# yl-jiang/YOLOSeries

Measured on AMD Instinct MI355X. Metric: images/sec (640x640) YOLOv5s train-step, higher is better.
Workload: dtype bf16; 1 GPU; YOLOv5s bf16 train step (fwd+loss+bwd+clip+SGD+EMA), batch 64/GPU x 640x640 synthetic COCO-80, random-init (BASELINE.json configs[1]); global_batch=64, parallelism=dp1

## Files before the change

include/yolohip.h:

```cpp
#ifndef YOLOHIP_H
#define YOLOHIP_H

#include <stddef.h>
#include <stdint.h>

#ifdef __cplusplus
extern "C" {
#endif

typedef void* yh_stream;
typedef uint16_t yh_bf16;

enum yh_status {
    YH_OK = 0,
    YH_EINVAL = -1,
    YH_ELAUNCH = -2,
    YH_EUNSUPPORTED = -3
};

const char* yh_last_error(void);
int yh_version(void);
int yh_device_cus(void);


// ... 88 lines not shown
                          const float* ws, int C, int64_t M, float* part, yh_stream stream);
int yh_bn_bwd_finalize(const float* part, int nblk, int C, int64_t M, const float* ws,
                       float* dgamma, float* dbeta, float* coef, yh_stream stream);
int yh_bn_silu_bwd_apply(const yh_bf16* ga, int ldga, const yh_bf16* y, int ldy,
                         const float* ws, const float* gamma, const float* coef,
                         int C, int64_t M, yh_bf16* gy, int ldgy,
                         yh_bf16* gres, int ldgres, int gres_accumulate, yh_stream stream);
#define YH_BN_MAX_PARTS 4
typedef struct yh_bn_part {
    float*         ws;
    int32_t        C;
    int32_t        ldo;
    yh_bf16*       out;
    const yh_bf16* ga;
    int32_t        ldga;
    int32_t        nblk;
    const float*   gamma;
    float*         coef;
    const float*   slab;
    int32_t        ldslab;
    float          eps;
    const float*   beta;
    float*         running_mean;
    float*         running_var;
    int64_t*       num_batches;
    float          momentum;
    int32_t        _pad;
    float*         dgamma;
    float*         dbeta;
} yh_bn_part;
int yh_bn_finalize_parts(const yh_bn_part* parts, int nparts, int64_t count, yh_stream stream);
int yh_bn_bwd_finalize_parts(const yh_bn_part* parts, int nparts, int64_t M, yh_stream stream);
int yh_bn_silu_apply_parts(const yh_bf16* y, int ldy, int64_t M, const yh_bn_part* parts, int nparts, yh_stream stream);
int yh_bn_silu_bwd_apply_parts(const yh_bf16* y, int ldy, int64_t M, const yh_bn_part* parts, int nparts,
                               yh_bf16* gy, int ldgy, yh_stream stream);
int yh_colsum(const yh_bf16* g, int ldg, int C, int64_t M, float* part, float* out, yh_stream stream);

int yh_maxpool5_fwd(const yh_bf16* x, int ldx, int B, int H, int W, int C,
                    yh_bf16* out, int ldo, int8_t* idx, yh_stream stream);
int yh_maxpool5_bwd(const yh_bf16* gout, int ldgo, const int8_t* idx, int B, int H, int W, int C,
                    yh_bf16* gin, int ldgi, int accumulate, yh_stream stream);
int yh_sppf_pool3_ok(int H, int W, int C);
int yh_sppf_pool3_fwd(const yh_bf16* x, int ldx, int B, int H, int W, int C, yh_bf16* o1, yh_bf16* o2, yh_bf16* o3, int ldo,
                      int8_t* i1, int8_t* i2, int8_t* i3, yh_stream stream);
int yh_sppf_pool3_bwd(const yh_bf16* g1, const yh_bf16* g2, const yh_bf16* g3, int ldg, const int8_t* i1, const int8_t* i2, const int8_t* i3,
                      int B, int H, int W, int C, yh_bf16* gx, int ldx, int accumulate, yh_stream stream);
int yh_upsample2_bwd(const yh_bf16* ghi, int ldh, int B, int Hlo, int Wlo, int C,
                     yh_bf16* glo, int ldl, int accumulate, yh_stream stream);
int yh_input_s2d(const float* x, int B, int Cin, int H, int W, yh_bf16* out, yh_stream stream);
int yh_fill_u32(void* p, uint32_t v, int64_t n_words, yh_stream stream);

int yh_pack_bf16(const float* src, const int32_t* idx, int64_t n, yh_bf16* dst, yh_stream stream);
int yh_gather_f32(const float* src, const int32_t* idx, int64_t n, float* dst, yh_stream stream);
int yh_sgd_step(float* p, const float* g, float* buf, const uint8_t* group, int64_t n,
                const float* lr, const float* wd, int ngroups, float momentum, int nesterov,
                int first_step, const float* grad_scale, yh_stream stream);
int yh_sgd_step_dev(float* p, const float* g, float* buf, const uint8_t* group, int64_t n,
                    const float* scal, int nesterov, const float* grad_scale, yh_stream stream);
int yh_ema_update_dev(float* ema, const float* p, int64_t n, const float* decay_dev, yh_stream stream);
int yh_ema_advance(int64_t* counter, float* decay, double ratio, double tau, yh_stream stream);
int yh_sumsq(const float* x, int64_t n, float* part, float* out, yh_stream stream);
int yh_clip_scale(const float* sumsq, float max_norm, float* out, yh_stream stream);
int yh_ema_update(float* ema, const float* p, int64_t n, float decay, yh_stream stream);

typedef struct yh_v5loss_desc {
    int32_t B, maxbox, num_class, num_anchor, num_stage;
    int32_t H[4], W[4];
    float   img_size0, img_size1;
    float   anchors[4][3][2];
    float   anchor_thr;
    float   cls_smooth, cls_pos_weight, cof_pos_weight;
    int32_t use_focal; float focal_gamma, focal_alpha;
    float   iou_scale, cof_scale, cls_scale;
    int32_t pred_is_f32;
    int32_t ldp[4];
    int32_t targets_xywhn;
} yh_v5loss_desc;

size_t yh_v5loss_ws_bytes(const yh_v5loss_desc* d);
int yh_v5_assign(const yh_v5loss_desc* d, const float* targets,
                 int32_t* count, float* tbox, int32_t* tidx, void* ws, yh_stream stream);
size_t yh_v5loss_saved_bytes(const yh_v5loss_desc* d);
int yh_v5_loss_fwd(const yh_v5loss_desc* d, const void* const* preds, const float* targets,
                   double* balances, float* result, void* saved, void* ws, yh_stream stream);
int yh_v5_loss_bwd(const yh_v5loss_desc* d, const void* const* preds, const float* gout,
                   const void* saved, void* const* gpreds, void* ws, yh_stream stream);

typedef struct yh_yolox_desc {
    int32_t B, maxbox, num_class, num_stage;
    int32_t H[4], W[4], ldp[4];
    int32_t pred_is_f32;
    float   img_size0;
    int32_t use_focal; float focal_gamma, focal_alpha;
    int32_t use_l1;
    float   iou_scale, cls_scale, cof_scale, l1_scale;
    float   cls_smooth, cls_pos_weight, cof_pos_weight;
    int32_t iou_type;
    int32_t topk; float center_radius;
    float   cls_cost_const;
} yh_yolox_desc;
size_t yh_yolox_saved_bytes(const yh_yolox_desc* d);
size_t yh_yolox_ws_bytes(const yh_yolox_desc* d);
int yh_yolox_layout(const yh_yolox_desc* d, int64_t* out8);
int yh_yolox_loss_fwd(const yh_yolox_desc* d, const void* const* preds, const float* targets_xywh,
                      double* balances, float* result, void* saved, void* ws, yh_stream stream);
int yh_yolox_loss_bwd(const yh_yolox_desc* d, const void* const* preds, const float* targets_xywh, const float* gout,
// ... 43 lines not shown
```

yoloseries_amd/_lib.py:

```python
import ctypes as C
import os
import subprocess

_HERE = os.path.dirname(os.path.abspath(__file__))
LIB_PATH = os.environ.get("YH_LIBRARY") or os.path.join(_HERE, "libyolohip.so")
CSRC_DIR = os.path.join(_HERE, "csrc")


class YoloHipError(RuntimeError):
    pass


class Seg(C.Structure):
    _fields_ = [("ptr", C.c_void_p), ("ld", C.c_int32), ("C", C.c_int32), ("ups", C.c_int32), ("_pad", C.c_int32)]


class ConvDesc(C.Structure):
    _fields_ = [
        ("seg", Seg * 2), ("nseg", C.c_int32), ("mode", C.c_int32),
        ("B", C.c_int32), ("Ho", C.c_int32), ("Wo", C.c_int32),
        ("Hi", C.c_int32), ("Wi", C.c_int32),
        ("KH", C.c_int32), ("KW", C.c_int32), ("stride", C.c_int32), ("pad", C.c_int32),
        ("w", C.c_void_p), ("N", C.c_int32), ("Npad", C.c_int32),
        ("bias", C.c_void_p), ("scale", C.c_void_p), ("shift", C.c_void_p),
# ... 82 lines not shown
class Cmd(C.Structure):
    _fields_ = [("op", C.c_int32), ("nslots", C.c_int32), ("stream", C.c_int32), ("reserved", C.c_int32),
                ("slots", C.c_uint64 * YH_CMD_SLOTS)]


YH_CONV_FWD, YH_CONV_DGRAD = 0, 1
YH_ACT_NONE, YH_ACT_SILU = 0, 1

_lib = None

_vp, _i32, _i64, _f32, _sz = C.c_void_p, C.c_int32, C.c_int64, C.c_float, C.c_size_t
_SIGS = {
    "yh_last_error": (C.c_char_p, []),
    "yh_version": (_i32, []),
    "yh_device_cus": (_i32, []),
    "yh_conv_stat_blocks": (_i32, [C.POINTER(ConvDesc)]),
    "yh_conv_igemm": (_i32, [C.POINTER(ConvDesc), _vp]),
    "yh_conv_wgrad": (_i32, [C.POINTER(WgradDesc), _vp]),
    "yh_conv_wgrad_ws_bytes": (C.c_size_t, [C.POINTER(WgradDesc)]),
    "yh_conv_wgrad_patch_ok": (_i32, [C.POINTER(WgradDesc)]),
    "yh_conv_wgrad_patch_name": (_i32, [C.POINTER(WgradDesc), C.c_char_p, _i32]),
    "yh_conv_wgrad_wave_tiles": (_i32, [C.POINTER(WgradDesc)]),
    "yh_conv_wgrad_wave_name": (C.c_char_p, [C.POINTER(WgradDesc)]),
    "yh_conv_wgrad_tiles": (_i32, [_i32, _i32]),
    "yh_conv_wgrad_tiles2": (_i32, [_i32, _i32, _i32]),
    "yh_conv_wgrad_kernel_name": (C.c_char_p, [_i32, _i32]),
    "yh_conv_wgrad_kernel_name2": (C.c_char_p, [_i32, _i32, _i32]),
    "yh_conv_bnr_rows": (_i32, [C.POINTER(ConvDesc)]),
    "yh_conv_kernel_name": (_i32, [C.POINTER(ConvDesc), C.c_char_p, _i32]),
    "yh_bn_finalize": (_i32, [_vp, _i32, _i32, _i32, _i64, _vp, _vp, _vp, _vp, _vp, _f32, _f32, _vp, _vp]),
    "yh_bn_fold": (_i32, [_vp, _vp, _vp, _vp, _f32, _i32, _vp, _vp, _vp]),
    "yh_bn_frozen": (_i32, [_vp, _vp, _vp, _vp, _f32, _i32, _vp, _vp]),
    "yh_bn_fold_batch": (_i32, [_vp, _i32, _vp]),
    "yh_bn_silu_apply": (_i32, [_vp, _i32, _vp, _i32, _i64, _vp, _i32, _vp, _i32, _vp]),
    "yh_ew_blocks": (_i32, [_i64]),
    "yh_bn_silu_bwd_reduce": (_i32, [_vp, _i32, _vp, _i32, _vp, _i32, _i64, _vp, _vp]),
    "yh_bn_bwd_finalize": (_i32, [_vp, _i32, _i32, _i64, _vp, _vp, _vp, _vp, _vp]),
    "yh_bn_finalize_parts": (_i32, [_vp, _i32, _i64, _vp]),
    "yh_bn_bwd_finalize_parts": (_i32, [_vp, _i32, _i64, _vp]),
    "yh_bn_silu_apply_parts": (_i32, [_vp, _i32, _i64, _vp, _i32, _vp]),
    "yh_bn_silu_bwd_apply_parts": (_i32, [_vp, _i32, _i64, _vp, _i32, _vp, _i32, _vp]),
    "yh_bn_silu_bwd_apply": (_i32, [_vp, _i32, _vp, _i32, _vp, _vp, _vp, _i32, _i64, _vp, _i32, _vp, _i32, _i32, _vp]),
    "yh_colsum": (_i32, [_vp, _i32, _i32, _i64, _vp, _vp, _vp]),
    "yh_maxpool5_fwd": (_i32, [_vp, _i32, _i32, _i32, _i32, _i32, _vp, _i32, _vp, _vp]),
    "yh_maxpool5_bwd": (_i32, [_vp, _i32, _vp, _i32, _i32, _i32, _i32, _vp, _i32, _i32, _vp]),
    "yh_sppf_pool3_ok": (_i32, [_i32, _i32, _i32]),
    "yh_sppf_pool3_fwd": (_i32, [_vp, _i32, _i32, _i32, _i32, _i32, _vp, _vp, _vp, _i32, _vp, _vp, _vp, _vp]),
    "yh_sppf_pool3_bwd": (_i32, [_vp, _vp, _vp, _i32, _vp, _vp, _vp, _i32, _i32, _i32, _i32, _vp, _i32, _i32, _vp]),
    "yh_upsample2_bwd": (_i32, [_vp, _i32, _i32, _i32, _i32, _i32, _vp, _i32, _i32, _vp]),
    "yh_input_s2d": (_i32, [_vp, _i32, _i32, _i32, _i32, _vp, _vp]),
    "yh_fill_u32": (_i32, [_vp, C.c_uint32, _i64, _vp]),
    "yh_pack_bf16": (_i32, [_vp, _vp, _i64, _vp, _vp]),
    "yh_gather_f32": (_i32, [_vp, _vp, _i64, _vp, _vp]),
    "yh_sgd_step": (_i32, [_vp, _vp, _vp, _vp, _i64, _vp, _vp, _i32, _f32, _i32, _i32, _vp, _vp]),
    "yh_sgd_step_dev": (_i32, [_vp, _vp, _vp, _vp, _i64, _vp, _i32, _vp, _vp]),
    "yh_ema_update_dev": (_i32, [_vp, _vp, _i64, _vp, _vp]),
    "yh_ema_advance": (_i32, [_vp, _vp, C.c_double, C.c_double, _vp]),
    "yh_sumsq": (_i32, [_vp, _i64, _vp, _vp, _vp]),
    "yh_clip_scale": (_i32, [_vp, _f32, _vp, _vp]),
    "yh_ema_update": (_i32, [_vp, _vp, _i64, _f32, _vp]),
    "yh_v5loss_ws_bytes": (_sz, [C.POINTER(V5LossDesc)]),
    "yh_v5loss_saved_bytes": (_sz, [C.POINTER(V5LossDesc)]),
    "yh_v5_assign": (_i32, [C.POINTER(V5LossDesc), _vp, _vp, _vp, _vp, _vp, _vp]),
    "yh_v5_loss_fwd": (_i32, [C.POINTER(V5LossDesc), C.POINTER(_vp), _vp, _vp, _vp, _vp, _vp, _vp]),
    "yh_v5_loss_bwd": (_i32, [C.POINTER(V5LossDesc), C.POINTER(_vp), _vp, _vp, C.POINTER(_vp), _vp, _vp]),
    "yh_yolox_saved_bytes": (_sz, [C.POINTER(YoloxDesc)]),
    "yh_yolox_ws_bytes": (_sz, [C.POINTER(YoloxDesc)]),
    "yh_yolox_layout": (_i32, [C.POINTER(YoloxDesc), _vp]),
    "yh_yolox_loss_fwd": (_i32, [C.POINTER(YoloxDesc), C.POINTER(_vp), _vp, _vp, _vp, _vp, _vp, _vp]),
    "yh_yolox_loss_bwd": (_i32, [C.POINTER(YoloxDesc), C.POINTER(_vp), _vp, _vp, _vp, C.POINTER(_vp), _vp]),
    "yh_iou_matrix": (_i32, [_vp, _i32, _vp, _i32, _f32, _vp, _vp]),
    "yh_iou_pairwise": (_i32, [_i32, _vp, _vp, _i32, _vp, _vp, _vp]),
    "yh_decode_full": (_i32, [C.POINTER(DecodeDesc), C.POINTER(_vp), _vp, _vp]),
    "yh_decode_filter": (_i32, [C.POINTER(DecodeDesc), C.POINTER(_vp), _f32, _f32, _vp, _vp, _i32, _vp, _vp]),
    "yh_decode_filter_ws_bytes": (C.c_size_t, [C.POINTER(DecodeDesc)]),
    "yh_filter_decoded": (_i32, [_vp, _i32, _i32, _i32, _f32, _f32, _i32, _vp, _vp, _i32, _vp]),
    "yh_exec_op": (_i32, [C.c_char_p, C.POINTER(_i32)]),
    "yh_exec": (_i32, [C.POINTER(Cmd), _i32, C.POINTER(_vp), _i32, C.POINTER(_i32)]),
    "yh_nms_ws_bytes": (_sz, [_i32, _i32]),
    "yh_nms_batched": (_i32, [_vp, _vp, _i32, _i32, _f32, _i32, _i32, _i32, _i32, _vp, _vp, _vp, _vp, _vp]),
}
EXPORTED_SYMBOLS = tuple(_SIGS.keys())


def build(force=False):
    if force:
        subprocess.run(["make", "-C", CSRC_DIR, "clean"], check=True, stdout=subprocess.DEVNULL)
    r = subprocess.run(["make", "-C", CSRC_DIR, "-j8"], stdout=subprocess.PIPE, stderr=subprocess.STDOUT, text=True)
    if r.returncode != 0:
        raise YoloHipError("building libyolohip.so failed:\n" + r.stdout[-4000:])
    return LIB_PATH


def lib():
    global _lib
    if _lib is not None:
        return _lib
    if not os.path.exists(LIB_PATH):
        raise YoloHipError(
            f"{LIB_PATH} not found: the HIP extension is required (run __graft_entry__.build() or "
            f"`make -C {CSRC_DIR}`); there is no CPU fallback for the product path.")
    import torch
    L = C.CDLL(LIB_PATH)
    missing = []
    for name, (res, args) in _SIGS.items():
        try:
# ... 22 lines not shown
```

yoloseries_amd/csrc/arena.hip:

```cpp
#include "common.h"
#include <stdarg.h>

namespace {
constexpr int TH = 256;
inline int grid_for(long n) {
    long g = (n + TH - 1) / TH;
    if (g > 4096) g = 4096;
    if (g < 1) g = 1;
    return (int)g;
}

__global__ void pack_bf16_kernel(const float* __restrict__ src, const int32_t* __restrict__ idx, long n, uint16_t* __restrict__ dst)
{
    const long n8 = ((reinterpret_cast<uintptr_t>(dst) | reinterpret_cast<uintptr_t>(idx)) & 15) ? 0 : n >> 3;
    for (long c = (long)blockIdx.x * blockDim.x + threadIdx.x; c < n8; c += (long)gridDim.x * blockDim.x) {
        const int4 j0 = *reinterpret_cast<const int4*>(idx + c * 8), j1 = *reinterpret_cast<const int4*>(idx + c * 8 + 4);
        const int j[8] = {j0.x, j0.y, j0.z, j0.w, j1.x, j1.y, j1.z, j1.w};
        float f[8];
#pragma unroll
        for (int e = 0; e < 8; ++e) f[e] = j[e] >= 0 ? src[j[e]] : 0.f;
        uint4 v;
        v.x = (uint32_t)f2bf(f[0]) | ((uint32_t)f2bf(f[1]) << 16);
        v.y = (uint32_t)f2bf(f[2]) | ((uint32_t)f2bf(f[3]) << 16);
        v.z = (uint32_t)f2bf(f[4]) | ((uint32_t)f2bf(f[5]) << 16);
        v.w = (uint32_t)f2bf(f[6]) | ((uint32_t)f2bf(f[7]) << 16);
        *reinterpret_cast<uint4*>(dst + c * 8) = v;
    }
    for (long i = n8 * 8 + (long)blockIdx.x * blockDim.x + threadIdx.x; i < n; i += (long)gridDim.x * blockDim.x) {
        int32_t j = idx[i];
        dst[i] = j >= 0 ? f2bf(src[j]) : (uint16_t)0;
    }
}
__global__ void gather_f32_kernel(const float* __restrict__ src, const int32_t* __restrict__ idx, long n, float* __restrict__ dst)
{
    const long n4 = ((reinterpret_cast<uintptr_t>(dst) | reinterpret_cast<uintptr_t>(idx)) & 15) ? 0 : n >> 2;
    for (long c = (long)blockIdx.x * blockDim.x + threadIdx.x; c < n4; c += (long)gridDim.x * blockDim.x) {
        const int4 j = *reinterpret_cast<const int4*>(idx + c * 4);
        float4 v;
        v.x = j.x >= 0 ? src[j.x] : 0.f; v.y = j.y >= 0 ? src[j.y] : 0.f; v.z = j.z >= 0 ? src[j.z] : 0.f; v.w = j.w >= 0 ? src[j.w] : 0.f;
        *reinterpret_cast<float4*>(dst + c * 4) = v;
    }
    for (long i = n4 * 4 + (long)blockIdx.x * blockDim.x + threadIdx.x; i < n; i += (long)gridDim.x * blockDim.x) {
        int32_t j = idx[i];
        dst[i] = j >= 0 ? src[j] : 0.f;
    }
}
__global__ void sgd_kernel(float* __restrict__ p, const float* __restrict__ g, float* __restrict__ buf,
                           const uint8_t* __restrict__ group, long n, const float* __restrict__ lr,
                           const float* __restrict__ wd, float momentum, int nesterov, int first,
                           const float* __restrict__ grad_scale)
{
    const float gs = grad_scale ? *grad_scale : 1.f;
    for (long i = (long)blockIdx.x * blockDim.x + threadIdx.x; i < n; i += (long)gridDim.x * blockDim.x) {
        int gi = group ? group[i] : 0;
        float pv = p[i];
        float gv = g[i] * gs + wd[gi] * pv;
        float b = first ? gv : momentum * buf[i] + gv;
        buf[i] = b;
        float upd = nesterov ? gv + momentum * b : b;
        p[i] = pv - lr[gi] * upd;
    }
}
__global__ void sgd_dev_kernel(float* __restrict__ p, const float* __restrict__ g, float* __restrict__ buf,
                               const uint8_t* __restrict__ group, long n, const float* __restrict__ scal, int nesterov,
                               const float* __restrict__ grad_scale)
{
    const float gs = grad_scale ? *grad_scale : 1.f;
    const float lr[3] = {scal[0], scal[1], scal[2]}, wd[3] = {scal[3], scal[4], scal[5]};
    const float momentum = scal[6];
    const bool first = scal[7] != 0.f;
    for (long i = (long)blockIdx.x * blockDim.x + threadIdx.x; i < n; i += (long)gridDim.x * blockDim.x) {
        int gi = group ? group[i] : 0;
        gi = gi > 2 ? 2 : gi;
        float pv = p[i];
        float gv = g[i] * gs + (gi == 0 ? wd[0] : (gi == 1 ? wd[1] : wd[2])) * pv;
        float b = first ? gv : momentum * buf[i] + gv;
        buf[i] = b;
        float upd = nesterov ? gv + momentum * b : b;
        p[i] = pv - (gi == 0 ? lr[0] : (gi == 1 ? lr[1] : lr[2])) * upd;
    }
}
__global__ void ema_dev_kernel(float* __restrict__ e, const float* __restrict__ p, long n, const float* __restrict__ decay_dev)
{
    const float decay = *decay_dev;
    for (long i = (long)blockIdx.x * blockDim.x + threadIdx.x; i < n; i += (long)gridDim.x * blockDim.x)
// ... 91 lines not shown
                       p, g, buf, group, (long)n, lr, wd, momentum, nesterov, first_step, grad_scale);
    YH_CHECK_LAUNCH("yh_sgd_step");
    return YH_OK;
}
extern "C" int yh_sgd_step_dev(float* p, const float* g, float* buf, const uint8_t* group, int64_t n,
                               const float* scal, int nesterov, const float* grad_scale, yh_stream stream)
{
    YH_CHECK_ARG(p && g && buf && scal && n >= 0, "yh_sgd_step_dev: bad args");
    if (n == 0) return YH_OK;
    hipLaunchKernelGGL(sgd_dev_kernel, dim3(grid_for(n)), dim3(TH), 0, (hipStream_t)stream, p, g, buf, group, (long)n, scal, nesterov, grad_scale);
    YH_CHECK_LAUNCH("yh_sgd_step_dev");
    return YH_OK;
}
extern "C" int yh_ema_update_dev(float* ema, const float* p, int64_t n, const float* decay_dev, yh_stream stream)
{
    YH_CHECK_ARG(ema && p && decay_dev && n >= 0, "yh_ema_update_dev: bad args");
    if (n == 0) return YH_OK;
    hipLaunchKernelGGL(ema_dev_kernel, dim3(grid_for(n)), dim3(TH), 0, (hipStream_t)stream, ema, p, (long)n, decay_dev);
    YH_CHECK_LAUNCH("yh_ema_update_dev");
    return YH_OK;
}
extern "C" int yh_ema_advance(int64_t* counter, float* decay, double ratio, double tau, yh_stream stream)
{
    YH_CHECK_ARG(counter && decay && tau > 0.0, "yh_ema_advance: bad args");
    hipLaunchKernelGGL(ema_advance_kernel, dim3(1), dim3(64), 0, (hipStream_t)stream, (long long*)counter, decay, ratio, tau);
    YH_CHECK_LAUNCH("yh_ema_advance");
    return YH_OK;
}
extern "C" int yh_sumsq(const float* x, int64_t n, float* part, float* out, yh_stream stream)
{
    YH_CHECK_ARG(x && part && out && n > 0, "yh_sumsq: bad args (part needs 4096 floats)");
    int nb = grid_for(n);
    hipLaunchKernelGGL(sumsq_part_kernel, dim3(nb), dim3(TH), 0, (hipStream_t)stream, x, (long)n, part);
    hipLaunchKernelGGL(sum_final_kernel, dim3(1), dim3(256), 0, (hipStream_t)stream, part, nb, out);
    YH_CHECK_LAUNCH("yh_sumsq");
    return YH_OK;
}
extern "C" int yh_ema_update(float* ema, const float* p, int64_t n, float decay, yh_stream stream)
{
    YH_CHECK_ARG(ema && p && n >= 0, "yh_ema_update: bad args");
    if (n == 0) return YH_OK;
    hipLaunchKernelGGL(ema_kernel, dim3(grid_for(n)), dim3(TH), 0, (hipStream_t)stream, ema, p, (long)n, decay);
    YH_CHECK_LAUNCH("yh_ema_update");
    return YH_OK;
}

extern "C" int yh_clip_scale(const float* sumsq, float max_norm, float* out, yh_stream stream)
{
    YH_CHECK_ARG(sumsq && out && max_norm > 0.f, "yh_clip_scale: bad args");
    hipLaunchKernelGGL(clip_scale_kernel, dim3(1), dim3(64), 0, (hipStream_t)stream, sumsq, max_norm, out);
    YH_CHECK_LAUNCH("yh_clip_scale");
    return YH_OK;
}
```

yoloseries_amd/engine/graph.py:

```python
import numpy as np
import torch

from .. import hipk
from .._lib import YoloHipError
from ..hipk import Slice
from . import flags as _flags
from .flags import BN_EPS_DEFAULT


def _rup(x, m):
    return ((x + m - 1) // m) * m


def plan_grad_buckets(marks, gsize, nbuckets):
    out, hi, last = [], gsize, gsize
    target = max(1, gsize // max(1, nbuckets))
    for i, (ci, lo) in enumerate(marks):
        if lo > last:
            raise YoloHipError("gradient arena is not laid out in forward op order")
        last = lo
        if hi - lo >= target or i == len(marks) - 1:
            lo_cut = 0 if i == len(marks) - 1 else lo
            out.append((ci, lo_cut, hi))
            hi = lo_cut
    return out


def _pick_bn(n):
    return 32 if n <= 32 else (64 if n <= 64 else 128)


class TBuf:

    def __init__(self, name, H, W, Cn, needs_grad=True):
        self.name, self.H, self.W, self.C = name, H, W, Cn
        self.needs_grad = needs_grad
        self.t = None
        self.g = None
        self.ginit = None


class Ref:

    def __init__(self, buf, coff=0, Cn=None, ups=0):
        self.buf, self.coff, self.C, self.ups = buf, coff, (buf.C - coff if Cn is None else Cn), ups

    def sl(self, grad=False):
        return Slice(self.buf.g if grad else self.buf.t, self.coff, self.C, self.ups)


class ConvOp:
    def __init__(self, name, segs, parts, k, stride, pad, Hi, Wi, kind, outs, res, focus=False):
        self.name, self.segs, self.parts = name, segs, parts
        self.k, self.stride, self.pad, self.Hi, self.Wi = k, stride, pad, Hi, Wi
        self.Ho = (Hi + 2 * pad - k) // stride + 1
        self.Wo = (Wi + 2 * pad - k) // stride + 1
        self.kind, self.outs, self.res, self.focus = kind, outs, res, focus
        self.Ctot = sum(s.C for s in segs)
        self.Ktot = k * k * self.Ctot
        self.part_N = [c.out_channels for c, _ in parts]
# ... 75 lines not shown
        op.y = self.buf(name + ".out", op.Ho, op.Wo, _rup(op.N, 8))
        op.y.is_head = True
        self.ops.append(op)
        return op

    def plain_multi(self, name, parts, segs):
        Hi, Wi = segs[0].buf.H, segs[0].buf.W
        c0 = parts[0][0]
        op = ConvOp(name, segs, [(c, None) for c, _ in parts], c0.kernel_size[0], c0.stride[0], c0.padding[0], Hi, Wi, 'plain', None, None)
        op.part_seg = [si for _, si in parts]
        op.y = self.buf(name + ".out", op.Ho, op.Wo, _rup(op.N, 8))
        op.y.is_head = True
        self.ops.append(op)
        return op

    def pool(self, name, src, dst):
        self.ops.append(PoolOp(name, src, dst))


class ParamPack:

    def __init__(self, module, ops, host_only=False):
        params = list(module.parameters())
        if not params:
            raise YoloHipError("model has no parameters")
        dev = params[0].device
        if dev.type != "cuda" and not host_only:
            raise YoloHipError("yoloseries_amd models run on an MI355X device only (no CPU path in the product); call .to('cuda') first")
        self.device = dev
        self.params = params
        if any(p.dtype != torch.float32 for p in params):
            raise YoloHipError("master parameters must be float32 (bf16 copies are made by the engine)")
        sizes = [p.numel() for p in params]
        offs = np.concatenate([[0], np.cumsum(sizes)]).astype(np.int64)
        self.n = int(offs[-1])
        fbufs = [b for b in module.buffers() if b.dtype == torch.float32]
        nb = sum(b.numel() for b in fbufs)
        self.nbuf = nb
        self.flat = self.fbuf = None
        if not host_only:
            flat = torch.empty(self.n, dtype=torch.float32, device=dev)
            for p, o in zip(params, offs[:-1]):
                flat[o:o + p.numel()].copy_(p.data.reshape(-1))
                p.data = flat[o:o + p.numel()].view(p.shape)
            self.flat = flat
            self.fbuf = torch.empty(max(nb, 1), dtype=torch.float32, device=dev)
            o = 0
            for b in fbufs:
                self.fbuf[o:o + b.numel()].copy_(b.data.reshape(-1))
                b.data = self.fbuf[o:o + b.numel()].view(b.shape)
                o += b.numel()
        self.off = {id(p): int(o) for p, o in zip(params, offs[:-1])}
        pack_idx, self.wloc = [], {}
        fpack_idx, self.bias_loc = [], {}
        fcur = 0
        cur = 0
        gcur = 0
        unpack = np.full(self.n, -1, dtype=np.int64)
        self.gloc, self.bn_g, self.bias_g = {}, {}, {}
        self.fused_ops = set()

        def widx(conv):
            w = conv.weight
            return self.off[id(w)] + np.arange(w.numel(), dtype=np.int64).reshape(tuple(w.shape))

        for op in ops:
            if not isinstance(op, ConvOp):
                continue
            part_seg = getattr(op, "part_seg", None)
            if part_seg is None:
                Wall = np.concatenate([widx(c) for c, _ in op.parts], axis=0)
            else:
                Wall = np.full((op.N, op.Ctot, op.k, op.k), -1, dtype=np.int64)
                seg_c0 = np.concatenate([[0], np.cumsum([sg.C for sg in op.segs])])
                r = 0
                for (conv, _), si in zip(op.parts, part_seg):
                    o = conv.out_channels
                    Wall[r:r + o, seg_c0[si]:seg_c0[si + 1]] = widx(conv)
                    r += o
            N = op.N
            if op.focus:
                n_, ci, kh6, kw6 = Wall.shape
                assert kh6 == 6 and kw6 == 6 and 4 * ci <= 16
                P = np.full((N, 3, 3, 16), -1, dtype=np.int64)
                for dy in range(2):
                    for dx in range(2):
                        for c in range(ci):
                            P[:, :, :, (dy * 2 + dx) * ci + c] = Wall[:, c, dy::2, dx::2]
                P = P.reshape(N, 9 * 16)
            else:
                P = Wall.transpose(0, 2, 3, 1).reshape(N, op.Ktot)
            Pp = np.full((op.Npad, op.Ktot), -1, dtype=np.int64)
            Pp[:N] = P
            self.wloc[(op.name, 'fwd')] = (cur, op.Npad, op.Ktot)
            pack_idx.append(Pp.reshape(-1)); cur += Pp.size
            pos = gcur + np.arange(N * op.Ktot, dtype=np.int64).reshape(N, op.Ktot)
            valid = P >= 0
            unpack[P[valid]] = pos[valid]
            self.gloc[op.name] = gcur
            gcur += _rup(N * op.Ktot, 8)
            if not op.focus:
                Nk = _rup(N, 8)
                Wk = Wall
                if Nk != N:
                    Wk = np.concatenate([Wall, np.full((Nk - N,) + Wall.shape[1:], -1, dtype=np.int64)], axis=0)
                c0 = 0
                for si, sg in enumerate(op.segs):
                    if sg.buf.needs_grad:
                        D = Wk[:, c0:c0 + sg.C].transpose(1, 2, 3, 0).reshape(sg.C, op.k * op.k * Nk)
                        Cp = _rup(sg.C, 128)
                        Dp = np.full((Cp, D.shape[1]), -1, dtype=np.int64)
                        Dp[:sg.C] = D
                        self.wloc[(op.name, 'dgrad', si)] = (cur, Cp, D.shape[1])
                        pack_idx.append(Dp.reshape(-1)); cur += Dp.size
                    c0 += sg.C
            if op.kind == 'plain':
                brow = np.full(_rup(N, 8), -1, dtype=np.int64)
                r = 0
                for conv, _ in op.parts:
                    if conv.bias is not None:
                        brow[r:r + conv.out_channels] = self.off[id(conv.bias)] + np.arange(conv.out_channels)
                        unpack[self.off[id(conv.bias)]:self.off[id(conv.bias)] + conv.out_channels] = gcur + r + np.arange(conv.out_channels)
                    r += conv.out_channels
                self.bias_loc[op.name] = fcur
                fpack_idx.append(brow); fcur += len(brow)
                self.bias_g[(op.name, 0)] = gcur
                gcur += _rup(N, 8)
            for pi, (conv, bn) in enumerate(op.parts):
                if op.kind == 'plain':
                    break
                if bn is not None and id(bn.weight) not in self.off:
                    self.fused_ops.add(op.name)
                elif bn is not None:
                    Cn = bn.weight.numel()
                    unpack[self.off[id(bn.weight)]:self.off[id(bn.weight)] + Cn] = gcur + np.arange(Cn)
                    unpack[self.off[id(bn.bias)]:self.off[id(bn.bias)] + Cn] = gcur + Cn + np.arange(Cn)
                    self.bn_g[(op.name, pi)] = (gcur, gcur + Cn)
                    gcur += _rup(2 * Cn, 8)
        if cur >= 2 ** 31 or gcur >= 2 ** 31:
            raise YoloHipError("parameter arena too large for int32 index maps")
        self.pack_idx_np = np.concatenate(pack_idx).astype(np.int32)
        self.unpack_idx_np = unpack.astype(np.int32)
        self.fpack_idx_np = np.concatenate(fpack_idx).astype(np.int32) if fpack_idx else None
        self.gsize = gcur
        if host_only:
            return
        self.pack_idx = torch.from_numpy(self.pack_idx_np).to(dev)
        self.unpack_idx = torch.from_numpy(self.unpack_idx_np).to(dev)
        self.wpack = torch.zeros(cur, dtype=torch.bfloat16, device=dev)
        self.fpack_idx = torch.from_numpy(self.fpack_idx_np).to(dev) if fpack_idx else None
        self.fpack = torch.zeros(max(fcur, 8), dtype=torch.float32, device=dev)
        self.gsize = gcur
        self.gpack = torch.zeros(max(gcur, 8), dtype=torch.float32, device=dev)
        self.packed_version = -1

    def valid_for(self, module):
        ps = list(module.parameters())
        return len(ps) == len(self.params) and all(a is b for a, b in zip(ps, self.params)) and \
            ps[0].data_ptr() == self.flat.data_ptr() and ps[0].device == self.device

    def still_valid(self):
        p0, p1 = self.params[0], self.params[-1]
        return p0.data_ptr() == self.flat.data_ptr() and p1.data_ptr() == self.flat.data_ptr() + 4 * (self.n - p1.numel())

    def repack(self):
        hipk.pack_bf16(self.flat, self.pack_idx, self.wpack)
        if self.fpack_idx is not None:
            hipk.gather_f32(self.flat, self.fpack_idx, self.fpack)

    def wptr(self, key):
        off, rows, K = self.wloc[key]
        return self.wpack.data_ptr() + 2 * off, rows, K

    def grads_to_params(self, views=True):
        flat_g = torch.empty(self.n, dtype=torch.float32, device=self.device)
        hipk.gather_f32(self.gpack, self.unpack_idx, flat_g)
        if not views:
            return flat_g, None
        outs, o = [], 0
        for p in self.params:
            outs.append(flat_g[o:o + p.numel()].view(p.shape))
            o += p.numel()
        return flat_g, outs
```

yoloseries_amd/hipk.py:

```python
import ctypes as C
from dataclasses import dataclass

import torch

from . import _lib
from ._lib import ConvDesc, Seg, WgradDesc, YH_ACT_NONE, YH_ACT_SILU, YH_CONV_DGRAD, YH_CONV_FWD, check, lib


def _st():
    return C.c_void_p(torch.cuda.current_stream().cuda_stream)


def _p(t, elem_off=0):
    if t is None:
        return None
    return C.c_void_p(t.data_ptr() + elem_off * t.element_size())


@dataclass
class Slice:
    buf: torch.Tensor
    coff: int
    C: int
    ups: int = 0
# ... 140 lines not shown

def bn_bwd_finalize_parts(parts, M):
    arr = _bn_parts(parts)
    check(lib().yh_bn_bwd_finalize_parts(arr, len(parts), M, _st()), "yh_bn_bwd_finalize_parts")


def bn_silu_apply_parts(y: Slice, M, parts):
    arr = _bn_parts(parts)
    check(lib().yh_bn_silu_apply_parts(y.ptr(), y.ld, M, arr, len(parts), _st()), "yh_bn_silu_apply_parts")


def bn_silu_bwd_apply_parts(y: Slice, M, parts, gy: Slice):
    arr = _bn_parts(parts)
    check(lib().yh_bn_silu_bwd_apply_parts(y.ptr(), y.ld, M, arr, len(parts), gy.ptr(), gy.ld, _st()), "yh_bn_silu_bwd_apply_parts")


def colsum(g: Slice, M, part, out):
    check(lib().yh_colsum(g.ptr(), g.ld, g.C, M, _p(part), _p(out), _st()), "yh_colsum")


def maxpool5_fwd(x: Slice, B, H, W, out: Slice, idx):
    check(lib().yh_maxpool5_fwd(x.ptr(), x.ld, B, H, W, x.C, out.ptr(), out.ld, _p(idx), _st()), "yh_maxpool5_fwd")


def maxpool5_bwd(gout: Slice, idx, B, H, W, gin: Slice, accumulate):
    check(lib().yh_maxpool5_bwd(gout.ptr(), gout.ld, _p(idx), B, H, W, gout.C, gin.ptr(), gin.ld, accumulate, _st()),
          "yh_maxpool5_bwd")


def upsample2_bwd(ghi: Slice, B, Hlo, Wlo, glo: Slice, accumulate):
    check(lib().yh_upsample2_bwd(ghi.ptr(), ghi.ld, B, Hlo, Wlo, ghi.C, glo.ptr(), glo.ld, accumulate, _st()),
          "yh_upsample2_bwd")


def input_s2d(x, out):
    B, Cin, H, W = x.shape
    check(lib().yh_input_s2d(_p(x), B, Cin, H, W, _p(out), _st()), "yh_input_s2d")


def fill_zero(t):
    nbytes = t.numel() * t.element_size()
    assert nbytes % 4 == 0
    check(lib().yh_fill_u32(_p(t), 0, nbytes // 4, _st()), "yh_fill_u32")


def pack_bf16(src, idx, dst):
    check(lib().yh_pack_bf16(_p(src), _p(idx), idx.numel(), _p(dst), _st()), "yh_pack_bf16")


def gather_f32(src, idx, dst):
    check(lib().yh_gather_f32(_p(src), _p(idx), idx.numel(), _p(dst), _st()), "yh_gather_f32")


def sgd_step(p, g, buf, group, lr, wd, momentum, nesterov, first, grad_scale=None):
    check(lib().yh_sgd_step(_p(p), _p(g), _p(buf), _p(group), p.numel(), _p(lr), _p(wd), lr.numel(), momentum,
                            int(nesterov), int(first), _p(grad_scale), _st()), "yh_sgd_step")


def sumsq(x, part, out):
    check(lib().yh_sumsq(_p(x), x.numel(), _p(part), _p(out), _st()), "yh_sumsq")


def ema_update(ema, p, decay):
    check(lib().yh_ema_update(_p(ema), _p(p), p.numel(), decay, _st()), "yh_ema_update")


def clip_scale(sumsq_t, max_norm, out):
    check(lib().yh_clip_scale(_p(sumsq_t), float(max_norm), _p(out), _st()), "yh_clip_scale")


def sgd_step_dev(p, g, buf, group, scal, nesterov, grad_scale=None):
    check(lib().yh_sgd_step_dev(_p(p), _p(g), _p(buf), _p(group), p.numel(), _p(scal), int(nesterov), _p(grad_scale), _st()), "yh_sgd_step_dev")


def ema_update_dev(ema, p, decay_dev):
    check(lib().yh_ema_update_dev(_p(ema), _p(p), p.numel(), _p(decay_dev), _st()), "yh_ema_update_dev")


def ema_advance(counter, decay, ratio, tau):
    check(lib().yh_ema_advance(_p(counter), _p(decay), float(ratio), float(tau), _st()), "yh_ema_advance")
```

Before: 5477 images/sec.

## Replace index-gather weight repack with structured tile-based LDS transpose kernel

The per-step weight repack (fp32 master weights to bf16 packed forward and dgrad layouts, plus the fp32 bias gather) used index gathers driven by large int32 index arrays. Now a host-built tile descriptor table lets a single kernel stage contiguous weight blocks in LDS, transpose them and write vectorized bf16 output. Irregular images fall back to index mapping, and the bias gather is folded into the same launch. This cuts index-array traffic, scattered reads and one launch, at the cost of a more complex descriptor-driven kernel whose LDS use and magic-number division must stay correct.

```diff
diff --git a/include/yolohip.h b/include/yolohip.h
--- a/include/yolohip.h
+++ b/include/yolohip.h
@@ -164,6 +164,8 @@
 
 int yh_pack_bf16(const float* src, const int32_t* idx, int64_t n, yh_bf16* dst, yh_stream stream);
 int yh_gather_f32(const float* src, const int32_t* idx, int64_t n, float* dst, yh_stream stream);
+int yh_pack_tiles(const float* src, const int32_t* tiles, int ntiles, const int32_t* idx, yh_bf16* dst,
+                  const int32_t* fidx, float* fdst, yh_stream stream);
 int yh_sgd_step(float* p, const float* g, float* buf, const uint8_t* group, int64_t n,
                 const float* lr, const float* wd, int ngroups, float momentum, int nesterov,
                 int first_step, const float* grad_scale, yh_stream stream);
diff --git a/yoloseries_amd/_lib.py b/yoloseries_amd/_lib.py
--- a/yoloseries_amd/_lib.py
+++ b/yoloseries_amd/_lib.py
@@ -158,6 +158,7 @@
     "yh_fill_u32": (_i32, [_vp, C.c_uint32, _i64, _vp]),
     "yh_pack_bf16": (_i32, [_vp, _vp, _i64, _vp, _vp]),
     "yh_gather_f32": (_i32, [_vp, _vp, _i64, _vp, _vp]),
+    "yh_pack_tiles": (_i32, [_vp, _vp, _i32, _vp, _vp, _vp, _vp, _vp]),
     "yh_sgd_step": (_i32, [_vp, _vp, _vp, _vp, _i64, _vp, _vp, _i32, _f32, _i32, _i32, _vp, _vp]),
     "yh_sgd_step_dev": (_i32, [_vp, _vp, _vp, _vp, _i64, _vp, _i32, _vp, _vp]),
     "yh_ema_update_dev": (_i32, [_vp, _vp, _i64, _vp, _vp]),
diff --git a/yoloseries_amd/csrc/arena.hip b/yoloseries_amd/csrc/arena.hip
--- a/yoloseries_amd/csrc/arena.hip
+++ b/yoloseries_amd/csrc/arena.hip
@@ -31,6 +31,75 @@
         dst[i] = j >= 0 ? f2bf(src[j]) : (uint16_t)0;
     }
 }
+constexpr int PT_WORDS = 16, PT_LDS = 4800;
+enum { PT_COPY_C = 0, PT_COPY_N = 1, PT_MAP = 2, PT_ZERO = 3, PT_F32 = 4 };
+__device__ __forceinline__ uint32_t pt_div(uint32_t x, uint32_t magic) { return magic ? __umulhi(x, magic) : x; }
+__global__ __launch_bounds__(TH) void pack_tiles_kernel(const float* __restrict__ src, const int32_t* __restrict__ tiles,
+                                                        const int32_t* __restrict__ idx, uint16_t* __restrict__ dst,
+                                                        const int32_t* __restrict__ fidx, float* __restrict__ fdst)
+{
+    __shared__ float lds[PT_LDS];
+    const int32_t* d = tiles + (long)blockIdx.x * PT_WORDS;
+    const int kind = d[0], tid = threadIdx.x;
+    const long dst_off = d[3];
+    const int VE = d[9];
+    const bool dst16 = (reinterpret_cast<uintptr_t>(dst) & 15) == 0;
+    if (kind == PT_MAP) {
+        for (int i = tid; i < VE; i += TH) {
+            const int32_t j = idx[dst_off + i];
+            dst[dst_off + i] = j >= 0 ? f2bf(src[j]) : (uint16_t)0;
+        }
+        return;
+    }
+    if (kind == PT_F32) {
+        for (int i = tid; i < VE; i += TH) {
+            const int32_t j = fidx[dst_off + i];
+            fdst[dst_off + i] = j >= 0 ? src[j] : 0.f;
+        }
+        return;
+    }
+    if (kind == PT_ZERO) {
+        if (dst16 && (dst_off & 7) == 0) {
+            for (int i = tid * 8; i + 8 <= VE; i += TH * 8) *reinterpret_cast<uint4*>(dst + dst_off + i) = make_uint4(0, 0, 0, 0);
+            for (int i = (VE & ~7) + tid; i < VE; i += TH) dst[dst_off + i] = 0;
+        } else {
+            for (int i = tid; i < VE; i += TH) dst[dst_off + i] = 0;
+        }
+        return;
+    }
+    const int NV = d[6], CV = d[7], T = d[8], VV = d[10], OE = d[11];
+    const long so = d[4], st = d[5], src_ns = d[2];
+    const uint32_t m_row = (uint32_t)d[12], m_nvec = (uint32_t)d[13], m_T = (uint32_t)d[14];
+    const int rowlen = CV * T, row = rowlen | 1;
+    const float* s = src + d[1];
+    for (int i = tid; i < NV * rowlen; i += TH) {
+        const int n = (int)pt_div((uint32_t)i, m_row), k = i - n * rowlen;
+        lds[n * row + k] = s[n * src_ns + k];
+    }
+    __syncthreads();
+    const int lv = kind == PT_COPY_C ? T : row, lo = kind == PT_COPY_C ? row : T;
+    const int nvec = (VE + 7) >> 3;
+    for (int it = tid; it < OE * T * nvec; it += TH) {
+        const int q = (int)pt_div((uint32_t)it, m_nvec), vg = it - q * nvec;
+        const int o = (int)pt_div((uint32_t)q, m_T), t = q - o * T;
+        const int v0 = vg * 8;
+        const long a = dst_off + o * so + t * st + v0;
+        const float* l = lds + o * lo + t;
+        uint16_t h[8];
+#pragma unroll
+        for (int e = 0; e < 8; ++e) h[e] = v0 + e < VV ? f2bf(l[(v0 + e) * lv]) : (uint16_t)0;
+        if (v0 + 8 <= VE && dst16 && (a & 7) == 0) {
+            uint4 w;
+            w.x = (uint32_t)h[0] | ((uint32_t)h[1] << 16); w.y = (uint32_t)h[2] | ((uint32_t)h[3] << 16);
+            w.z = (uint32_t)h[4] | ((uint32_t)h[5] << 16); w.w = (uint32_t)h[6] | ((uint32_t)h[7] << 16);
+            *reinterpret_cast<uint4*>(dst + a) = w;
+        } else {
+#pragma unroll
+            for (int e = 0; e < 8; ++e)
+                if (v0 + e < VE) dst[a + e] = h[e];
+        }
+    }
+}
 __global__ void gather_f32_kernel(const float* __restrict__ src, const int32_t* __restrict__ idx, long n, float* __restrict__ dst)
 {
     const long n4 = ((reinterpret_cast<uintptr_t>(dst) | reinterpret_cast<uintptr_t>(idx)) & 15) ? 0 : n >> 2;
@@ -228,3 +297,13 @@
     YH_CHECK_LAUNCH("yh_clip_scale");
     return YH_OK;
 }
+
+extern "C" int yh_pack_tiles(const float* src, const int32_t* tiles, int ntiles, const int32_t* idx, yh_bf16* dst,
+                             const int32_t* fidx, float* fdst, yh_stream stream)
+{
+    YH_CHECK_ARG(src && tiles && idx && dst && ntiles >= 0, "yh_pack_tiles: bad args");
+    if (ntiles == 0) return YH_OK;
+    hipLaunchKernelGGL(pack_tiles_kernel, dim3(ntiles), dim3(TH), 0, (hipStream_t)stream, src, tiles, idx, (uint16_t*)dst, fidx, fdst);
+    YH_CHECK_LAUNCH("yh_pack_tiles");
+    return YH_OK;
+}
diff --git a/yoloseries_amd/engine/graph.py b/yoloseries_amd/engine/graph.py
--- a/yoloseries_amd/engine/graph.py
+++ b/yoloseries_amd/engine/graph.py
@@ -6,6 +6,7 @@
 from ..hipk import Slice
 from . import flags as _flags
 from .flags import BN_EPS_DEFAULT
+from .packtiles import build_tiles
 
 
 def _rup(x, m):
@@ -187,6 +188,7 @@
                 o += b.numel()
         self.off = {id(p): int(o) for p, o in zip(params, offs[:-1])}
         pack_idx, self.wloc = [], {}
+        images = []
         fpack_idx, self.bias_loc = [], {}
         fcur = 0
         cur = 0
@@ -228,6 +230,11 @@
             Pp = np.full((op.Npad, op.Ktot), -1, dtype=np.int64)
             Pp[:N] = P
             self.wloc[(op.name, 'fwd')] = (cur, op.Npad, op.Ktot)
+            rows0 = np.concatenate([[0], np.cumsum([c.out_channels for c, _ in op.parts])])
+            wparts = [(self.off[id(c.weight)], int(r0), c.out_channels) for (c, _), r0 in zip(op.parts, rows0)]
+            regular = not op.focus and part_seg is None
+            images.append({"kind": "fwd", "dst": cur, "Npad": op.Npad, "Ctot": op.Ctot, "T": op.k * op.k, "N": N, "parts": wparts}
+                          if regular else {"kind": "map", "dst": cur, "size": Pp.size})
             pack_idx.append(Pp.reshape(-1)); cur += Pp.size
             pos = gcur + np.arange(N * op.Ktot, dtype=np.int64).reshape(N, op.Ktot)
             valid = P >= 0
@@ -247,6 +254,8 @@
                         Dp = np.full((Cp, D.shape[1]), -1, dtype=np.int64)
                         Dp[:sg.C] = D
                         self.wloc[(op.name, 'dgrad', si)] = (cur, Cp, D.shape[1])
+                        images.append({"kind": "dgrad", "dst": cur, "Cp": Cp, "C": sg.C, "c0": c0, "Call": op.Ctot, "T": op.k * op.k,
+                                       "Nk": Nk, "N": N, "parts": wparts} if regular else {"kind": "map", "dst": cur, "size": Dp.size})
                         pack_idx.append(Dp.reshape(-1)); cur += Dp.size
                     c0 += sg.C
             if op.kind == 'plain':
@@ -278,8 +287,10 @@
         self.unpack_idx_np = unpack.astype(np.int32)
         self.fpack_idx_np = np.concatenate(fpack_idx).astype(np.int32) if fpack_idx else None
         self.gsize = gcur
+        self.tiles_np, self.mapped_images = build_tiles(images, self.pack_idx_np, self.n, fcur)
         if host_only:
             return
+        self.tiles = torch.from_numpy(self.tiles_np).to(dev)
         self.pack_idx = torch.from_numpy(self.pack_idx_np).to(dev)
         self.unpack_idx = torch.from_numpy(self.unpack_idx_np).to(dev)
         self.wpack = torch.zeros(cur, dtype=torch.bfloat16, device=dev)
@@ -299,9 +310,7 @@
         return p0.data_ptr() == self.flat.data_ptr() and p1.data_ptr() == self.flat.data_ptr() + 4 * (self.n - p1.numel())
 
     def repack(self):
-        hipk.pack_bf16(self.flat, self.pack_idx, self.wpack)
-        if self.fpack_idx is not None:
-            hipk.gather_f32(self.flat, self.fpack_idx, self.fpack)
+        hipk.pack_tiles(self.flat, self.tiles, self.pack_idx, self.wpack, self.fpack_idx, self.fpack)
 
     def wptr(self, key):
         off, rows, K = self.wloc[key]
diff --git a/yoloseries_amd/engine/packtiles.py b/yoloseries_amd/engine/packtiles.py
--- /dev/null
+++ b/yoloseries_amd/engine/packtiles.py
@@ -0,0 +1,158 @@
+import numpy as np
+
+WORDS = 16
+COPY_C, COPY_N, MAP, ZERO, F32 = 0, 1, 2, 3, 4
+LDS_FLOATS = 4800
+RANGE = 4096
+_TARGET = 4608
+
+
+def _magic(d):
+    assert 1 <= d < 65536
+    return 0 if d == 1 else (1 << 32) // d + 1
+
+
+def _range_tiles(kind, off, length):
+    return [[kind, 0, 0, o, 0, 0, 0, 0, 1, min(RANGE, off + length - o), 0, 0, 0, 0, 0, 0] for o in range(off, off + length, RANGE)]
+
+
+def _copy_tile(kind, src_off, src_ns, dst_off, so, st, NV, CV, T, VE, VV, OE):
+    assert NV * ((CV * T) | 1) <= LDS_FLOATS
+    return [kind, src_off, src_ns, dst_off, so, st, NV, CV, T, VE, VV, OE, _magic(CV * T), _magic((VE + 7) // 8), _magic(T), 0]
+
+
+def expected_map(img):
+    if img["kind"] == "fwd":
+        Npad, Ctot, T = img["Npad"], img["Ctot"], img["T"]
+        m = np.full((Npad, T, Ctot), -1, dtype=np.int64)
+        for src_off, r0, o in img["parts"]:
+            n, t, c = np.meshgrid(np.arange(o), np.arange(T), np.arange(Ctot), indexing="ij")
+            m[r0:r0 + o] = src_off + (n * Ctot + c) * T + t
+        return m.reshape(-1)
+    Cp, C, c0, Call, T, Nk = img["Cp"], img["C"], img["c0"], img["Call"], img["T"], img["Nk"]
+    m = np.full((Cp, T, Nk), -1, dtype=np.int64)
+    for src_off, r0, o in img["parts"]:
+        c, t, n = np.meshgrid(np.arange(C), np.arange(T), np.arange(o), indexing="ij")
+        m[:C, :, r0:r0 + o] = src_off + (n * Call + c0 + c) * T + t
+    return m.reshape(-1)
+
+
+def image_size(img):
+    if img["kind"] == "fwd":
+        return img["Npad"] * img["T"] * img["Ctot"]
+    if img["kind"] == "dgrad":
+        return img["Cp"] * img["T"] * img["Nk"]
+    return img["size"]
+
+
+def _fwd_tiles(img):
+    d0, Npad, Ctot, T, N = img["dst"], img["Npad"], img["Ctot"], img["T"], img["N"]
+    K = T * Ctot
+    CB = min(Ctot, 64)
+    NB = max(1, min(64, _TARGET // (CB * T)))
+    out = []
+    for src_off, r0, o in img["parts"]:
+        for n0 in range(0, o, NB):
+            nv = min(NB, o - n0)
+            for c0 in range(0, Ctot, CB):
+                cv = min(CB, Ctot - c0)
+                out.append(_copy_tile(COPY_C, src_off + (n0 * Ctot + c0) * T, Ctot * T, d0 + (r0 + n0) * K + c0, K, Ctot,
+                                      nv, cv, T, cv, cv, nv))
+    if Npad > N:
+        out += _range_tiles(ZERO, d0 + N * K, (Npad - N) * K)
+    return out
+
+
+def _dgrad_tiles(img):
+    d0, Cp, C, cs, Call, T, Nk, N = img["dst"], img["Cp"], img["C"], img["c0"], img["Call"], img["T"], img["Nk"], img["N"]
+    NB = 64
+    CB = max(1, min(C, 72 // T if T > 1 else 64))
+    out = []
+    for pi, (src_off, r0, o) in enumerate(img["parts"]):
+        last_part = pi == len(img["parts"]) - 1
+        for n0 in range(0, o, NB):
+            nv = min(NB, o - n0)
+            ne = nv + (Nk - N if last_part and n0 + nv == o else 0)
+            for c0 in range(0, C, CB):
+                cv = min(CB, C - c0)
+                out.append(_copy_tile(COPY_N, src_off + (n0 * Call + cs + c0) * T, Call * T, d0 + c0 * T * Nk + r0 + n0, T * Nk, Nk,
+                                      nv, cv, T, ne, nv, cv))
+    if Cp > C:
+        out += _range_tiles(ZERO, d0 + C * T * Nk, (Cp - C) * T * Nk)
+    return out
+
+
+def build_tiles(images, pack_idx, n_src, n_fpack=0):
+    tiles, cur, mapped = [], 0, 0
+    for img in images:
+        size = image_size(img)
+        assert img["dst"] == cur
+        ok = img["kind"] in ("fwd", "dgrad") and img["T"] * min(img.get("Ctot", 1), 64) <= _TARGET
+        if ok and img["kind"] == "fwd":
+            parts = img["parts"]
+            ok = [r0 for _, r0, _ in parts] == list(np.cumsum([0] + [o for _, _, o in parts[:-1]])) and sum(o for _, _, o in parts) == img["N"]
+        ok = ok and np.array_equal(expected_map(img), pack_idx[cur:cur + size])
+        if ok:
+            tiles += _fwd_tiles(img) if img["kind"] == "fwd" else _dgrad_tiles(img)
+        else:
+            tiles += _range_tiles(MAP, cur, size)
+            mapped += 1
+        cur += size
+    assert cur == len(pack_idx)
+    if n_fpack:
+        tiles += _range_tiles(F32, 0, n_fpack)
+    t = np.asarray(tiles, dtype=np.int64).reshape(-1, WORDS)
+    cp = t[t[:, 0] <= COPY_N]
+    if len(cp):
+        assert (cp[:, 1] >= 0).all() and (cp[:, 1] + (cp[:, 6] - 1) * cp[:, 2] + cp[:, 7] * cp[:, 8] <= n_src).all()
+        assert (cp[:, 3] >= 0).all() and (cp[:, 3] + (cp[:, 11] - 1) * cp[:, 4] + (cp[:, 8] - 1) * cp[:, 5] + cp[:, 9] <= cur).all()
+    rg = t[(t[:, 0] == MAP) | (t[:, 0] == ZERO)]
+    assert len(rg) == 0 or ((rg[:, 3] >= 0).all() and (rg[:, 3] + rg[:, 9] <= cur).all())
+    assert (t[:, 12:15] < 2 ** 32).all()
+    return t.astype(np.uint32).view(np.int32).reshape(-1, WORDS), mapped
+
+
+def emulate(tiles, src, pack_idx, fpack_idx=None):
+    out = np.zeros(len(pack_idx), dtype=np.float32)
+    hits = np.zeros(len(pack_idx), dtype=np.int32)
+    fout = None if fpack_idx is None else np.full(len(fpack_idx), np.nan, dtype=np.float32)
+
+    def div(x, m):
+        return x if m == 0 else (x * m) >> 32
+
+    for d in tiles.view(np.uint32).astype(np.int64):
+        kind, so_, ns, do_, so, st, NV, CV, T, VE, VV, OE, m_row, m_nvec, m_T = d[:15]
+        if kind in (MAP, ZERO):
+            sl = slice(do_, do_ + VE)
+            j = pack_idx[sl]
+            out[sl] = np.where(j >= 0, src[np.maximum(j, 0)], 0.0) if kind == MAP else 0.0
+            hits[sl] += 1
+            continue
+        if kind == F32:
+            j = fpack_idx[do_:do_ + VE]
+            fout[do_:do_ + VE] = np.where(j >= 0, src[np.maximum(j, 0)], 0.0)
+            continue
+        rowlen = CV * T
+        row = rowlen | 1
+        lds = np.full(LDS_FLOATS, np.nan, dtype=np.float32)
+        i = np.arange(NV * rowlen, dtype=np.int64)
+        n = div(i, m_row)
+        k = i - n * rowlen
+        assert (n == i // rowlen).all()
+        lds[n * row + k] = src[so_ + n * ns + k]
+        lv, lo = (T, row) if kind == COPY_C else (row, T)
+        nvec = (VE + 7) // 8
+        it = np.arange(OE * T * nvec, dtype=np.int64)
+        q = div(it, m_nvec)
+        vg = it - q * nvec
+        o = div(q, m_T)
+        t = q - o * T
+        assert (q == it // nvec).all() and (o == q // T).all()
+        for e in range(8):
+            v = vg * 8 + e
+            w = v < VE
+            a = (do_ + o * so + t * st + v)[w]
+            val = np.where(v < VV, lds[np.minimum(v, max(VV - 1, 0)) * lv + o * lo + t], 0.0)[w]
+            out[a] = val
+            np.add.at(hits, a, 1)
+    return out, hits, fout
diff --git a/yoloseries_amd/hipk.py b/yoloseries_amd/hipk.py
--- a/yoloseries_amd/hipk.py
+++ b/yoloseries_amd/hipk.py
@@ -216,6 +216,10 @@
     check(lib().yh_gather_f32(_p(src), _p(idx), idx.numel(), _p(dst), _st()), "yh_gather_f32")
 
 
+def pack_tiles(src, tiles, idx, dst, fidx, fdst):
+    check(lib().yh_pack_tiles(_p(src), _p(tiles), tiles.shape[0], _p(idx), _p(dst), _p(fidx), _p(fdst), _st()), "yh_pack_tiles")
+
+
 def sgd_step(p, g, buf, group, lr, wd, momentum, nesterov, first, grad_scale=None):
     check(lib().yh_sgd_step(_p(p), _p(g), _p(buf), _p(group), p.numel(), _p(lr), _p(wd), lr.numel(), momentum,
                             int(nesterov), int(first), _p(grad_scale), _st()), "yh_sgd_step")
```

Measured after the change: 5486 images/sec, median of 3. No clear change (+0.2%).
